# foobaz/pngloss

Measured on AMD Instinct MI355X. Metric: Mpixels/s (filter+quantise path), 4096x4096 RGBA8 s=19; bit-exact vs ref, higher is better.
Workload: dtype u8

## Files before the change

pngloss_amd/csrc/pl_seg_core.h:

```cpp
#ifndef PL_SEG_CORE_H
#define PL_SEG_CORE_H

#include <stdint.h>
#include <stddef.h>
#include <string.h>

#include "pl_result.h"

#if defined(__HIPCC__)
#define PLS_HD __host__ __device__ __forceinline__
#else
#define PLS_HD inline
#endif

#if defined(__HIP_DEVICE_COMPILE__)
#define PLS_THREADS(tid, nt) for (int tid = (int)threadIdx.x, pls_once_ = 1; pls_once_ && tid < (int)(nt); pls_once_ = 0)
#define PLS_SYNC() __syncthreads()
#define PLS_ATOMIC_ADD(p, v) atomicAdd((p), (v))
#define PLS_ATOMIC_MIN(p, v) atomicMin((p), (v))
#define PLS_ATOMIC_OR(p, v) atomicOr((p), (v))
#define PLS_ATOMIC_CAS(p, cmp, v) atomicCAS((p), (cmp), (v))
#define PLS_ATOMIC_ADD_RET(p, v) atomicAdd((p), (v))
#define PLS_ATOMIC_EXCH(p, v) atomicExch((p), (v))
#define PLS_ATOMIC_ADD64(p, v) atomicAdd((unsigned long long *)(p), (unsigned long long)(v))
// ... 92 lines not shown
#define SEG_UNC_SEEDS_OF(unit) ((unit) == 1 ? SEG_UNC_SEEDS1 : SEG_UNC_SEEDS)
#ifndef SEG_UNT
#define SEG_UNT 512
#endif
#define SEG_UPOOL SEG_UNT
#define SEG_GRP 16
#define SEG_VGRP 8
#define SEG_VGRP_UNITS 16
#ifndef SEG_TPARTS_BATCH
#define SEG_TPARTS_BATCH 1
#endif
#define SEG_VGRP_OF(tparts) ((tparts) == SEG_TPARTS_BATCH ? SEG_VGRP_UNITS : SEG_VGRP)
#define SEG_TPARTS 4
#define SEG_COMMIT_W 256
#define SEG_CTL_IMG_OF(P) (SEG_NFILT * (P).tparts)
#define SEG_PARTS 4
#define SEG_PL (SEG_L / SEG_PARTS)
#define SEG_NSP 256
#define SEG_NS_MAX 1024
#define SEG_TOFF 384
#define SEG_TN 768
#define SEG_TBL_WORDS (4 * SEG_TN + 128)
#define SEG_INVALID 0xFFFFu
#define SEG_NOFAIL 0xFFFFFFFFu
#define SEG_MAGIC 0x5E6C0DE1u
#define SEG_MAX_RESTARTS 12
#define SEG_NG_BURST 16
#define SEG_MAX_WIDTH (1u << 20)
#define SEG_THREADS 1024
#define SEG_CHAIN_THREADS 1024
#define SEG_CHAIN_THREADS_UNIT 256
#define SEG_REPLAY_THREADS (SEG_GRP * SEG_L)
// ... 600 lines not shown
    case 3: return seg_run_fast<3, TRX>(px, pstride, n, st, tw, cls, g, lut);
    case 4: return seg_run_fast<4, TRX>(px, pstride, n, st, tw, cls, g, lut);
    default: return seg_run_fast<0, TRX>(px, pstride, n, st, tw, cls, g, lut);
    }
}
PLS_HD int seg_run_fast_f(int f, bool trx, const SegPix *px, int pstride, int n, SegState &st, seg_lds_cu32 tw, seg_lds_cu8 cls, const SegGeo &g, seg_lds_cu32 lut)
{
    return trx ? seg_run_fast_t<true>(f, px, pstride, n, st, tw, cls, g, lut) : seg_run_fast_t<false>(f, px, pstride, n, st, tw, cls, g, lut);
}

#define SEG_K1 4
#ifndef SEG_K1_ONE_CHUNK
#define SEG_K1_ONE_CHUNK 4
#endif
PLS_HD int seg_k1(int ns) { return ns <= SEG_NSP ? SEG_K1_ONE_CHUNK : SEG_K1; }
#define SEG_HT 512
template <int NT>
PLS_HD void seg_enum_body(const SegJob &j, const SegParams &P, const SegCtlView &cv, int par, int f, int seg, int chalf, unsigned char *smem)
{
    if (cv.finished || cv.active != 1) return;
    const uint32_t W = j.W, bpp = j.bpp;
    constexpr int NCH = NT / SEG_NSP;
    const int c0 = chalf * NCH;
    if ((uint32_t)c0 >= bpp) return;
    const uint32_t x0 = (uint32_t)seg * SEG_L;
    if (x0 >= W) return;
    if (cv.start_x && x0 <= cv.start_x) return;
    uint32_t *tw = (uint32_t *)smem;
    SegPix *px = (SegPix *)(smem + SEG_TBL_WORDS * 4);
    uint32_t *lut = (uint32_t *)(px + (SEG_L + 1) * 4);
// ... 90 lines not shown
    PLS_THREADS(tid, NT) {
        uint32_t Dc[NCH];
        for (int k = 0; k < NCH; k++) Dc[k] = trflag[1 + k] < SEG_NSP ? trflag[1 + k] : SEG_NSP;
        int lc = 0, i = tid;
        uint32_t D = Dc[0];
        PLS_UNROLL
        for (int k = 0; k + 1 < NCH; k++) if (lc == k && (uint32_t)i >= Dc[k]) { i -= (int)Dc[k]; lc = k + 1; D = Dc[k + 1]; }
        const int c = c0 + lc;
        if (tid < NCH && (uint32_t)(c0 + tid) < bpp) j.dcnt[((size_t)f * j.nseg + seg) * 4 + c0 + tid] = trflag[1 + tid] < SEG_NSP ? trflag[1 + tid] : SEG_NSP;
        if ((uint32_t)c < bpp && (uint32_t)i < D) {
            const uint32_t key = uniq[lc * SEG_NSP + i];
            SegState st;
            st.left = (int)(key & 255u); st.cn = seg_sext8((int)(key >> 8)); st.th = seg_sext8((int)(key >> 16));
            uint32_t out = SEG_INVALID;
            const size_t slot = (((size_t)f * j.nseg + seg) * 4 + c) * SEG_NSP + i;
            int bad = seg_run_fast_f(f, trx, px + (1 + K1) * 4 + c, 4, SEG_PL - K1, st, SEG_LDS_CU32(tw), SEG_LDS_CU8(tw + 4 * SEG_TN), G, SEG_LDS_CU32(lut));
            for (int part = 1; part < SEG_PARTS; part++) {
                j.rck[slot * (SEG_PARTS - 1) + (part - 1)] = bad ? 0xFFFFFFFFu : seg_state_pack(st);
                bad |= seg_run_fast_f(f, trx, px + (1 + part * SEG_PL) * 4 + c, 4, SEG_PL, st, SEG_LDS_CU32(tw), SEG_LDS_CU8(tw + 4 * SEG_TN), G, SEG_LDS_CU32(lut));
            }
            if (!bad) out = seg_state_encode(P, px[SEG_L * 4 + c], st);
            j.rout[slot] = (uint16_t)out;
            j.rst[slot] = bad ? 0xFFFFFFFFu : seg_state_pack(st);
        }
        if (prof && tid == 0) {
            te[3] = PLS_CLOCK(); te[4] = te[3];
            for (int q = 0; q < PLR_SEG_ENUM_PHASES; q++) { PLS_ATOMIC_MAX(&j.result[PLR_SEG_ENUM_MAX + q], (int32_t)(te[q + 1] - te[q])); PLS_ATOMIC_ADD((uint32_t *)&j.result[PLR_SEG_ENUM_SUM + q], (uint32_t)(te[q + 1] - te[q])); }
            PLS_ATOMIC_ADD((uint32_t *)&j.result[PLR_SEG_ENUM_RUNS], 1u);
            PLS_ATOMIC_ADD((uint32_t *)&j.result[PLR_SEG_ENUM_STATES], trflag[1] + trflag[2] + trflag[3] + trflag[4]);
        }
    }
}

#define SEG_SM_ENUM_SEEDED(nt) (SEG_TBL_WORDS * 4 + (SEG_KIN + SEG_L + 1) * 4 * 8 + 2048 + 32 + 4 * SEG_EH_WORDS * 4 + 4 * SEG_EH_WORDS * 2 + 4 * SEG_NSP * 4 + (nt) * 4 + 128)
// ... 166 lines not shown
    }
    PLS_THREADS(tid, NT) {
        uint32_t Dc[NCH];
        for (int k = 0; k < NCH; k++) Dc[k] = trflag[1 + k] < SEG_NSP ? trflag[1 + k] : SEG_NSP;
        int lc = 0, i = tid;
        uint32_t D = Dc[0];
        PLS_UNROLL
        for (int k = 0; k + 1 < NCH; k++) if (lc == k && (uint32_t)i >= Dc[k]) { i -= (int)Dc[k]; lc = k + 1; D = Dc[k + 1]; }
        const int c = c0 + lc;
        if (tid < NCH && (uint32_t)(c0 + tid) < bpp) j.dcnt[((size_t)f * j.nseg + seg) * 4 + c0 + tid] = trflag[1 + tid] < SEG_NSP ? trflag[1 + tid] : SEG_NSP;
        if ((uint32_t)c < bpp && (uint32_t)i < D) {
            SegState st = seg_eh_state(uniq[lc * SEG_NSP + i]);
            const size_t slot = (((size_t)f * j.nseg + seg) * 4 + c) * SEG_NSP + i;
            const SegPix *ps = px + (nrun + 1) * 4 + c;
            int bad = 0;
            for (int part = 0; part < SEG_PARTS; part++) {
                if (part) j.rck[slot * (SEG_PARTS - 1) + (part - 1)] = bad ? 0xFFFFFFFFu : seg_state_pack(st);
                bad |= seg_run_fast_f(f, trx, ps + part * SEG_PL * 4, 4, SEG_PL, st, SEG_LDS_CU32(tw), SEG_LDS_CU8(tw + 4 * SEG_TN), G, SEG_LDS_CU32(lut));
            }
            j.rst[slot] = bad ? 0xFFFFFFFFu : seg_state_pack(st);
        }
        if (prof && tid == 0) {
            te[3] = PLS_CLOCK(); te[4] = te[3];
            for (int q = 0; q < PLR_SEG_ENUM_PHASES; q++) { PLS_ATOMIC_MAX(&j.result[PLR_SEG_ENUM_MAX + q], (int32_t)(te[q + 1] - te[q])); PLS_ATOMIC_ADD((uint32_t *)&j.result[PLR_SEG_ENUM_SUM + q], (uint32_t)(te[q + 1] - te[q])); }
            PLS_ATOMIC_ADD((uint32_t *)&j.result[PLR_SEG_ENUM_RUNS], 1u);
            PLS_ATOMIC_ADD((uint32_t *)&j.result[PLR_SEG_ENUM_STATES], two_stage ? 2u * (trflag[1] + trflag[2]) : trflag[1] + trflag[2] + trflag[3] + trflag[4]);
        }
    }
}

template <int NT>
PLS_HD void seg_enum_small_body(const SegJob &j, const SegParams &P, const SegCtlView &cv, int par, int f, int seg0, unsigned char *smem)
{
// ... 22 lines not shown
        for (int q = 0; q < NTW; q++) { const int i = tid + q * NT; if (i < SEG_TBL_WORDS) tw[i] = vt[q]; }
        if (tid < 512) lut[tid] = vl;
        if (tid < NSEGS * SEG_L) {
            seg_pix_split4(px + tid * 4, vp, bpp, (uint32_t)seg0 * SEG_L + (uint32_t)tid, W);
            if ((bpp & 1u) == 0u && (px[tid * 4 + (bpp - 1u)].w >> 24)) PLS_ATOMIC_OR(trflag, 1u);
        }
    }
    PLS_SYNC();
    const bool trx = *trflag != 0u;
    PLS_THREADS(tid, NT) {
        const int sl = tid / (4 * SEG_NSS), c = (tid / SEG_NSS) & 3, i = tid % SEG_NSS;
        const uint32_t seg = (uint32_t)seg0 + (uint32_t)sl, x0 = seg * SEG_L;
        if (seg < j.nseg && x0 < W && (x0 > cv.start_x || cv.start_x == 0) && (uint32_t)c < bpp && i < P.ns_small) {
            SegState st;
            uint32_t out = SEG_INVALID;
            const size_t slot = (((size_t)f * j.nseg + seg) * 4 + c) * SEG_NSP + i;
            if (seg_small_decode(P, i, st)) {
                int bad = 0;
                for (int part = 0; part < SEG_PARTS; part++) {
                    if (part) j.rck[slot * (SEG_PARTS - 1) + (part - 1)] = bad ? 0xFFFFFFFFu : seg_state_pack(st);
                    bad |= seg_run_fast_f(f, trx, px + (sl * SEG_L + part * SEG_PL) * 4 + c, 4, SEG_PL, st, SEG_LDS_CU32(tw), SEG_LDS_CU8(tw + 4 * SEG_TN), G, SEG_LDS_CU32(lut));
                }
                if (!bad) out = seg_small_encode(P, st);
            } else {
                for (int part = 1; part < SEG_PARTS; part++) j.rck[slot * (SEG_PARTS - 1) + (part - 1)] = 0xFFFFFFFFu;
            }
            j.maps[(((size_t)f * j.nseg + seg) * 4 + c) * (size_t)P.nsp + i] = (uint16_t)i;
            j.rout[(((size_t)f * j.nseg + seg) * 4 + c) * SEG_NSP + i] = (uint16_t)out;
            j.rst[(((size_t)f * j.nseg + seg) * 4 + c) * SEG_NSP + i] = out == SEG_INVALID ? 0xFFFFFFFFu : seg_state_pack(st);
            if (i == 0) j.dcnt[((size_t)f * j.nseg + seg) * 4 + c] = (uint32_t)P.ns_small;
        }
    }
}

#ifndef SEG_UNC_SMALL
#define SEG_UNC_SMALL (SEG_UNIT <= 3 ? 20 : (SEG_UNIT <= 4 ? 15 : (SEG_UNIT <= 6 ? 10 : 7)))
#endif
#define SEG_UNC_SMALL_OF(unit) ((unit) == SEG_UNIT ? SEG_UNC_SMALL : (SEG_UNC_SMALL < 20 ? SEG_UNC_SMALL : 20))
#define SEG_UNPX (SEG_UNC_SMALL * (SEG_UNIT * SEG_L + 1))
#define SEG_UN_K1MAX 4
// ... 9 lines not shown
        uint32_t m = bits[w];
        if (w == (a >> 5)) m &= 0xFFFFFFFFu << (a & 31u);
        if (w == ((b - 1u) >> 5) && (b & 31u)) m &= 0xFFFFFFFFu >> (32u - (b & 31u));
        n += (uint32_t)__builtin_popcount(m);
    }
    return n;
}
template <int LANES, int UNIT, int NC, bool SEEDS = false>
PLS_HD void seg_enum_unit_body(const SegJob &j, const SegParams &P, const SegCtlView &cv, int par, int f, int grp, unsigned char *smem)
{
    if (cv.finished || cv.active != 1) return;
    constexpr int NT = SEG_UNT, HT = 2 * LANES;
    constexpr int CPR = NT / LANES < NC ? NT / LANES : NC;
    constexpr int ROUNDS = (NC + CPR - 1) / CPR;
    constexpr uint32_t E = UNIT, UL = E * SEG_L, NPX = UL + 1;
    static_assert(CPR * HT <= 2 * SEG_UNT && CPR * LANES <= SEG_UNT && NC <= 24 && NC * (UNIT * SEG_L + 1) <= SEG_UNPX, "hash tables, per-turn lists, pixel records and the bookkeeping words are sized for this");
    const uint32_t W = j.W, bpp = j.bpp, nseg = j.nseg, nunit = (nseg + E - 1) / E, ncombo = nunit * bpp;
    const uint32_t q0 = (uint32_t)grp * NC;
    if (q0 >= ncombo) return;
    const uint32_t sx = cv.start_x;
    { const uint32_t ql = seg_umin(q0 + NC, ncombo) - 1u; if (sx && (ql / bpp) * UL <= sx) return; }
    constexpr uint32_t NP1 = SEEDS ? SEG_SEED_KMAX + 1 : SEG_UN_K1MAX + 1;
    uint32_t *tw = (uint32_t *)smem;
    uint32_t *lut = tw + SEG_TBL_WORDS;
    uint32_t *pool = lut + 512;
    SegPix *px1_std = (SegPix *)(pool + SEG_UPOOL);
    uint32_t *misc = (uint32_t *)(px1_std + SEG_UNC_SMALL * (SEG_UN_K1MAX + 1));
    uint32_t *ht = misc + 128;
    uint16_t *dense = (uint16_t *)(ht + 2 * SEG_UNT);
    uint32_t *uniqr = (uint32_t *)(dense + 2 * SEG_UNT);
// ... 207 lines not shown
                for (uint32_t sg = u * E; sg < seg_umin(u * E + E, nseg); sg++) j.dcnt[((size_t)f * nseg + sg) * 4 + c] = D;
            }
        }
        if ((uint32_t)tid < total) {
            int k = 0;
            PLS_UNROLL
            for (int q = 1; q < NC; q++) k += (uint32_t)tid >= misc[32 + q] ? 1 : 0;
            const uint32_t i = (uint32_t)tid - misc[32 + k], cq = q0 + (uint32_t)k, u = cq / bpp, c = cq % bpp;
            const uint32_t key = pool[tid];
            SegState st;
            st.left = (int)(key & 255u); st.cn = seg_sext8((int)(key >> 8)); st.th = seg_sext8((int)(key >> 16));
            const SegPix *pk = px + (size_t)k * NPX;
            const uint32_t sg0 = u * E, nsg = seg_umin(E, nseg - sg0);
            const size_t slot = (((size_t)f * nseg + sg0) * 4 + c) * SEG_NSP + i;
            int bad = 0;
            for (int part = 0; part < SEG_PARTS; part++) {
                if (part) j.rck[slot * (SEG_PARTS - 1) + (part - 1)] = bad ? 0xFFFFFFFFu : seg_state_pack(st);
                const int skip = part == 0 ? K1 : 0;
                bad |= seg_run_fast_f(f, trx, pk + 1 + part * SEG_PL + skip, 1, SEG_PL - skip, st, SEG_LDS_CU32(tw), SEG_LDS_CU8(tw + 4 * SEG_TN), G, SEG_LDS_CU32(lut));
            }
            const uint32_t ps0 = bad ? 0xFFFFFFFFu : seg_state_pack(st);
            j.rst[slot] = ps0;
            SEG_DEBUG_STATE(f, (long)cv.y * 100000 + (long)cq, 0, i, ps0);
            if (nsg == 1u) j.rout[slot] = (uint16_t)(bad ? (uint32_t)SEG_INVALID : seg_any_encode(P, f, pk[SEG_L], st));
            pool[tid] = nsg > 1u ? ps0 : 0xFFFFFFFFu;
        }
    }
    if (prof) { PLS_SYNC(); te[3] = PLS_CLOCK(); }
    if (E > 1u) {
        PLS_SYNC();
        PLS_THREADS(tid, NT) {
            const uint32_t total = misc[32 + NC];
            if ((uint32_t)tid < total) {
                const uint32_t ps = pool[tid];
// ... 36 lines not shown
        }
        PLS_SYNC();
        PLS_THREADS(tid, NT) {
            const uint32_t total2 = misc[64 + NC];
            if ((uint32_t)tid < total2) {
                int k = 0;
                PLS_UNROLL
                for (int q = 1; q < NC; q++) k += (uint32_t)tid >= misc[64 + q] ? 1 : 0;
                const uint32_t i = (uint32_t)tid - misc[64 + k], cq = q0 + (uint32_t)k, u = cq / bpp, c = cq % bpp;
                SegState st = seg_state_unpack(pool2[misc[32 + k] + i]);
                const SegPix *pk = px + (size_t)k * NPX;
                const uint32_t sg0 = u * E, nsg = seg_umin(E, nseg - sg0);
                int bad = 0;
                for (uint32_t sl = 1; sl < nsg; sl++) {
                    const size_t slot = (((size_t)f * nseg + sg0 + sl) * 4 + c) * SEG_NSP + i;
                    for (int part = 0; part < SEG_PARTS; part++) {
                        if (part) j.rck[slot * (SEG_PARTS - 1) + (part - 1)] = bad ? 0xFFFFFFFFu : seg_state_pack(st);
                        bad |= seg_run_fast_f(f, trx, pk + 1 + sl * SEG_L + part * SEG_PL, 1, SEG_PL, st, SEG_LDS_CU32(tw), SEG_LDS_CU8(tw + 4 * SEG_TN), G, SEG_LDS_CU32(lut));
                    }
                    j.rst[slot] = bad ? 0xFFFFFFFFu : seg_state_pack(st);
                    SEG_DEBUG_STATE(f, (long)cv.y * 100000 + (long)cq, sl, i, bad ? 0xFFFFFFFFu : seg_state_pack(st));
                    if (sl + 1 == nsg) j.rout[slot] = (uint16_t)(bad ? (uint32_t)SEG_INVALID : seg_any_encode(P, f, pk[(sl + 1) * SEG_L], st));
                }
            }
        }
    }
    if (prof) {
        PLS_SYNC();
        PLS_THREADS(tid, NT) {
            if (tid == 0) {
                te[4] = PLS_CLOCK();
                for (int q = 0; q < PLR_SEG_ENUM_PHASES; q++) { PLS_ATOMIC_MAX(&j.result[PLR_SEG_ENUM_MAX + q], (int32_t)(te[q + 1] - te[q])); PLS_ATOMIC_ADD((uint32_t *)&j.result[PLR_SEG_ENUM_SUM + q], (uint32_t)(te[q + 1] - te[q])); }
                PLS_ATOMIC_ADD((uint32_t *)&j.result[PLR_SEG_ENUM_RUNS], 1u);
// ... 7 lines not shown
{
    return seeds != 0 && P.seed_n > 0 && !seg_is_small(P, f) && cv.start_x == 0u && j.nbreak * 16u <= cv.y + 128u;
}

PLS_HD void seg_load_frozen(const SegJob &j, int par, int f, uint32_t *Hf, uint32_t *rank, int tid, int nt)
{
    for (int b = tid; b < 256; b += nt) {
        Hf[b] = j.H0[par * 256 + b] + j.base[((size_t)par * SEG_NFILT + f) * 256 + b];
        rank[b] = j.orig_rank[f * 256 + b];
    }
}

PLS_HD void seg_cnt_add(uint32_t *cnt, int bin, uint32_t v) { PLS_ATOMIC_ADD(&cnt[bin >> 2], v << (8 * (bin & 3))); }
PLS_HD uint32_t seg_cnt_get(const uint32_t *cnt, int bin) { return (cnt[bin >> 2] >> (8 * (bin & 3))) & 255u; }
static_assert(SEG_L * 4 <= 255, "a segment's bump count of a bin fits a byte");
PLS_HD void seg_walk(int f, const SegPix *px, int pstride, uint32_t xa, uint32_t xe, SegState &st, seg_lds_cu32 tw, seg_lds_cu32 lut, const uint32_t *Hf,
                     const uint32_t *rank, const SegGeo &G, const uint32_t *lut_g, int bleed, uint32_t *out, uint32_t *cnt)
{
    const SegState st0 = st;
    int bad = 0;
    const seg_lds_cu8 cls = SEG_LDS_CU8(tw + 4 * SEG_TN);
    for (uint32_t x = xa; x < xe; x++) {
        uint32_t w;
        const SegPix &p = px[(size_t)(x - xa) * pstride];
        switch (f) {
        case 1: w = seg_step_fast<1, true>(p, st, bad, tw, cls, G, lut); break;
        case 2: w = seg_step_fast<2, true>(p, st, bad, tw, cls, G, lut); break;
        case 3: w = seg_step_fast<3, true>(p, st, bad, tw, cls, G, lut); break;
        case 4: w = seg_step_fast<4, true>(p, st, bad, tw, cls, G, lut); break;
        default: w = seg_step_fast<0, true>(p, st, bad, tw, cls, G, lut); break;
        }
        if (out) out[(size_t)(x - xa) * 4] = w;
        if (cnt) seg_cnt_add(cnt, seg_cand_bin(w), 1u);
    }
    if (seg_bad(bad)) {
        if (cnt && out) for (uint32_t x = xa; x < xe; x++) seg_cnt_add(cnt, seg_cand_bin(out[(size_t)(x - xa) * 4]), 0u - 1u);
        st = st0;
        for (uint32_t x = xa; x < xe; x++) {
            const uint32_t w = seg_step_scan(f, px[(size_t)(x - xa) * pstride], st, Hf, nullptr, rank, G, lut_g, bleed);
            if (out) out[(size_t)(x - xa) * 4] = w;
            if (cnt) seg_cnt_add(cnt, seg_cand_bin(w), 1u);
        }
    }
}

template <int NT, bool UNITS>
PLS_HD void seg_first_body(const SegJob &j, const SegParams &P, const SegCtlView &cv, int par, int f, unsigned char *smem)
{
    const SegCtl &ctl = j.ctl[par];
    if (cv.finished || cv.active != 1) return;
    const uint32_t W = j.W, bpp = j.bpp, nseg = j.nseg;
    const uint32_t sx = cv.start_x;
    if (sx >= W || sx == 0) return;
    const uint32_t first = sx / SEG_L;
    if (first + 1 >= nseg) return;
    const uint32_t E = UNITS ? seg_unit_of(P, f) : 1u, ulast = seg_umin((first / E) * E + E - 1u, nseg - 1u);
// ... 513 lines not shown
template <int RNT>
PLS_HD void seg_replay_body(const SegJob &j, const SegParams &P, const SegCtlView &cv, int par, int f, int grp, unsigned char *smem)
{
    const SegCtl &ctl = j.ctl[par];
    if (cv.finished) return;
    const bool lazy = f == 0 && cv.active == 2;
    if (!lazy && cv.active != 1) return;
    const uint32_t W = j.W, bpp = j.bpp, nseg = j.nseg;
    const uint32_t sx = cv.start_x;
    const uint32_t first = sx / SEG_L;
    const uint32_t seg0 = (uint32_t)grp * SEG_GRP, x0g = seg0 * SEG_L;
    const bool walk = !lazy && sx < W && seg0 + SEG_GRP > first;
    uint32_t *Hf = (uint32_t *)smem, *rank = Hf + 256, *lut = Hf + 512, *tw = Hf + 1024;
    SegPix *px = (SegPix *)(tw + SEG_TBL_WORDS);
    uint32_t *cnt = (uint32_t *)(px + SEG_GRP * SEG_L * 4);
    uint32_t *lane = cnt + SEG_GRP * 64;
    uint32_t *cwl = lane + SEG_GRP * SEG_PARTS * 4 * 2;
    uint32_t *oaL = cwl + SEG_REPLAY_THREADS * 4;
    uint32_t *rm = tw;
    uint32_t *red = rm + 768;
    uint32_t *h0s = red + 16;
    const uint32_t y = cv.y;
    const uint32_t *row = seg_row_orig(j, y), *nab = y ? j.img + (size_t)(y - 1u) * W : nullptr, *e0g = seg_e0(j, y);
    const uint32_t *oab = y ? seg_row_orig(j, y - 1u) : nullptr;
    const SegGeo G = seg_geo((int)cv.s);
    const bool adaptive = !j.row_filters || y == 0;
    PLS_THREADS(tid, RNT) {
        const bool walker = walk && tid < SEG_GRP * SEG_PARTS * 4;
        const int sl = tid / (SEG_PARTS * 4), part = (tid >> 2) % SEG_PARTS, c = tid & 3;
        const uint32_t sg = seg0 + (uint32_t)sl;
        const bool live = walker && sg < nseg && sg >= first && (uint32_t)c < bpp;
        const size_t sc = ((size_t)f * nseg + (live ? sg : 0u)) * 4 + c;
        const uint32_t d = live ? (uint32_t)j.dnout[sc] : SEG_INVALID;
        constexpr int NTW = (SEG_TBL_WORDS + RNT - 1) / RNT;
        uint32_t vt[NTW], vl = 0, vh = 0, vb = 0, vr = 0;
        PLS_UNROLL
        for (int q = 0; q < NTW; q++) { const int i = tid + q * RNT; vt[q] = (walk && i < SEG_TBL_WORDS) ? j.tables[(size_t)f * SEG_TBL_WORDS + i] : 0u; }
        if (walk && tid < 512) vl = P.lut_a[tid];
        if (walk && tid < 256) { vh = j.H0[par * 256 + tid]; vb = j.base[((size_t)par * SEG_NFILT + f) * 256 + tid]; vr = j.orig_rank[f * 256 + tid]; }
        const bool pixlane = tid < SEG_REPLAY_THREADS;
        const uint32_t x = pixlane ? x0g + (uint32_t)tid : W;
        const SegPixRaw vp = seg_pix_fetch(row, nab, e0g, x, W);
        const uint32_t voa = (!lazy && oab && x < W) ? oab[x] : 0u;
        uint32_t voa0 = 0, vol0 = 0;
        SegVec16 vw, vw0; vw.a = vw.b = vw.c = vw.d = 0u; vw0 = vw;
        if (!lazy && tid == 0 && x0g) { voa0 = oab ? oab[x0g - 1] : 0u; vol0 = row[x0g - 1]; if (x0g <= sx) vw0 = *(const SEG_AS_GLB SegVec16 *)(j.cand + ((size_t)f * W + x0g - 1) * 4); }
        if (!lazy && x < W && (x < sx || !walk)) vw = *(const SEG_AS_GLB SegVec16 *)(j.cand + ((size_t)f * W + x) * 4);
        uint32_t ck[SEG_PARTS - 1], ent = 0;
        PLS_UNROLL
        for (int q = 0; q < SEG_PARTS - 1; q++) ck[q] = 0xFFFFFFFFu;
        if (live) {
            if (d != SEG_INVALID && d < SEG_NSP) {
                PLS_UNROLL
                for (int q = 0; q < SEG_PARTS - 1; q++) ck[q] = j.rck[(sc * SEG_NSP + d) * (SEG_PARTS - 1) + q];
            }
            if (part == 0) ent = sg == first ? ctl.state[f][c] : j.entry[sc];
        }
        uint32_t st0 = 0, range = 0xFFFFFFFFu;
        if (live) {
            const uint32_t x0 = sg * SEG_L, xend = (uint32_t)seg_min((int)(x0 + SEG_L), (int)W);
            bool mine = part == 0;
            uint32_t xa = sg == first ? sx : x0;
            if (part == 0) st0 = ent;
            else {
                uint32_t ckp = 0xFFFFFFFFu;
                PLS_UNROLL
                for (int q = 0; q < SEG_PARTS - 1; q++) if (q == part - 1) ckp = ck[q];
                if (ckp != 0xFFFFFFFFu && x0 + (uint32_t)part * SEG_PL < xend && x0 + (uint32_t)part * SEG_PL > xa) { mine = true; st0 = ckp; xa = x0 + (uint32_t)part * SEG_PL; }
            }
            if (mine) {
                uint32_t xe = xend;
                PLS_UNROLL
                for (int q = SEG_PARTS - 1; q >= 1; q--)
                    if (q > part && ck[q - 1] != 0xFFFFFFFFu && x0 + (uint32_t)q * SEG_PL < xend && x0 + (uint32_t)q * SEG_PL > xa) xe = x0 + (uint32_t)q * SEG_PL;
                range = (xa - x0g) | ((xe - x0g) << 16);
                SEG_DEBUG_COUNT(part ? 1 : 0, xe - xa);
            }
        }
        if (tid < SEG_GRP * SEG_PARTS * 4) { lane[2 * tid] = st0; lane[2 * tid + 1] = range; }
        if (walk) {
            PLS_UNROLL
            for (int q = 0; q < NTW; q++) { const int i = tid + q * RNT; if (i < SEG_TBL_WORDS) tw[i] = vt[q]; }
            if (tid < 512) lut[tid] = vl;
            if (tid < 256) { Hf[tid] = vh + vb; rank[tid] = vr; }
            for (int i = tid; i < SEG_GRP * 64; i += RNT) cnt[i] = 0u;
        }
        if (pixlane) {
            seg_pix_split4(px + tid * 4, vp, bpp, x, W);
            oaL[tid + 1] = voa;
            cwl[tid * 4 + 0] = vw.a; cwl[tid * 4 + 1] = vw.b; cwl[tid * 4 + 2] = vw.c; cwl[tid * 4 + 3] = vw.d;
        }
        if (tid == 0) {
            oaL[0] = voa0; oaL[SEG_REPLAY_THREADS + 1] = vol0;
            oaL[SEG_REPLAY_THREADS + 2] = (vw0.a & 255u) | ((vw0.b & 255u) << 8) | ((vw0.c & 255u) << 16) | ((vw0.d & 255u) << 24);
        }
    }
    PLS_SYNC();
    if (walk) {
        PLS_THREADS(tid, RNT) {
            if (tid < SEG_GRP * SEG_PARTS * 4 && lane[2 * tid + 1] != 0xFFFFFFFFu) {
                const int sl = tid / (SEG_PARTS * 4), c = tid & 3;
                SegState st = seg_state_unpack(lane[2 * tid]);
                const uint32_t ra = lane[2 * tid + 1] & 0xffffu, re = lane[2 * tid + 1] >> 16;
                seg_walk(f, px + ra * 4 + c, 4, x0g + ra, x0g + re, st, SEG_LDS_CU32(tw), SEG_LDS_CU32(lut), Hf, rank, G, lut, P.bleed, cwl + ra * 4 + c, cnt + sl * 64);
            }
        }
        PLS_SYNC();
    }
    SegAcc &A = j.acc[par];
    PLS_THREADS(tid, RNT) { if (tid < 16) red[tid] = tid == 14 ? (0x80000000u ^ (uint32_t)(-(1 << 30))) : (tid == 15 ? (0x80000000u ^ (uint32_t)(1 << 30)) : 0u); }
    PLS_SYNC();
    {
        PLS_THREADS(tid, RNT) {
            if (walk && tid >= RNT - SEG_REPLAY_THREADS && tid < RNT - SEG_REPLAY_THREADS + 256) {
                const int b = tid - (RNT - SEG_REPLAY_THREADS);
                uint32_t tot = 0, cvs[SEG_GRP];
                PLS_UNROLL
                for (int sl = 0; sl < SEG_GRP; sl++) cvs[sl] = seg_cnt_get(cnt + sl * 64, b);
                PLS_UNROLL
                for (int sl = 0; sl < SEG_GRP; sl++) {
                    const uint32_t sg = seg0 + (uint32_t)sl;
                    if (sg < nseg && sg >= first) { j.segcnt[((size_t)f * nseg + sg) * 256 + b] = (uint16_t)cvs[sl]; tot += cvs[sl]; }
                }
                j.grpcnt[((size_t)f * j.ngrp + grp) * 256 + b] = tot;
            }
            const uint32_t x = (!lazy && tid < SEG_REPLAY_THREADS) ? x0g + (uint32_t)tid : W;
            uint64_t derr = 0; uint32_t hs[SEG_NFILT] = { 0, 0, 0, 0, 0 };
            if (x < W) {
                SegVec16 w; w.a = cwl[tid * 4 + 0]; w.b = cwl[tid * 4 + 1]; w.c = cwl[tid * 4 + 2]; w.d = cwl[tid * 4 + 3];
                if (walk && x >= sx) *(SEG_AS_GLB SegVec16 *)(j.cand + ((size_t)f * W + x) * 4) = w;
                uint32_t lw[4];
                if (tid) { PLS_UNROLL for (int c = 0; c < 4; c++) lw[c] = cwl[(tid - 1) * 4 + c] & 255u; }
                else {
                    uint32_t l0 = 0;
                    if (x0g && x0g <= sx) l0 = oaL[SEG_REPLAY_THREADS + 2];
                    else if (x0g) {
                        for (uint32_t c = 0; c < bpp; c++) l0 |= (walk ? (lane[2 * c] & 255u) : 0u) << (8 * c);
                        j.grpleft[(size_t)f * j.ngrp + grp] = l0;
                    }
                    PLS_UNROLL for (int c = 0; c < 4; c++) lw[c] = (l0 >> (8 * c)) & 255u;
                }
                const uint32_t wv[4] = { w.a, w.b, w.c, w.d };
                const uint32_t oav4 = oaL[tid + 1], odv4 = oaL[tid];
                for (uint32_t c = 0; c < bpp; c++) {
                    const int sh = 8 * (int)c;
                    const SegPix pc = px[tid * 4 + c];
                    const int back = (int)(wv[c] & 255u), nl = x ? (int)lw[c] : 0;
                    const int ov = (int)(pc.w & 255u), nav = (int)((pc.w >> 8) & 255u), ndv = (int)((pc.w >> 16) & 255u);
                    const int olv = tid ? (int)(px[(tid - 1) * 4 + c].w & 255u) : (int)((oaL[SEG_REPLAY_THREADS + 1] >> sh) & 255u);
                    const int oav = (int)((oav4 >> sh) & 255u), odv = (int)((odv4 >> sh) & 255u);
                    const int da = (oav - ov) - (nav - back), dd = (odv - ov) - (ndv - back), dl = (olv - ov) - (nl - back);
                    const uint32_t wgt = (bpp <= 2 && c == 0) ? 3u : 1u;
                    derr += (uint64_t)(wgt * (uint32_t)(da * da + dd * dd + dl * dl));
                    if (adaptive) {
                        const int preds[SEG_NFILT] = { 0, nl, nav, (nav + nl) >> 1, seg_paeth(nav, ndv, nl) };
                        for (int g = 0; g < SEG_NFILT; g++) { const int bb = (back - preds[g]) & 255; hs[g] += (uint32_t)(bb < 128 ? bb : 256 - bb); }
                    }
                }
            }
            derr = (uint64_t)pls_wave_sum_u32((uint32_t)derr);
            if (adaptive) for (int g = 0; g < SEG_NFILT; g++) hs[g] = pls_wave_sum_u32(hs[g]);
            if (PLS_WAVE_LEADER(tid)) {
                PLS_ATOMIC_ADD64((uint64_t *)&red[0], derr);
                if (adaptive) for (int g = 0; g < SEG_NFILT; g++) PLS_ATOMIC_ADD(&red[2 + g], hs[g]);
            }
        }
    }
    int R = -1;
    if (f == 0 && j.rowmm) {
        const int32_t *rmm = seg_rowmm(j, y);
        PLS_THREADS(tid, RNT) {
// ... 30 lines not shown
                        if (pc.w >> 24) hmax = h0s[0];
                        else hmax = rm[seg_min(seg_max((int)(pc.w & 255u) + pc.e0, -256), 511) + 256];
                        const uint32_t fr = hmax + rowbumps;
                        lb += 33u + (uint32_t)__builtin_clz(fr ? fr : 1u);
                    }
                }
                lb = pls_wave_sum_u64(lb);
                if (PLS_WAVE_LEADER(tid) && lb) PLS_ATOMIC_ADD64((uint64_t *)&red[10], lb);
            }
        }
    }
    PLS_SYNC();
    PLS_THREADS(tid, RNT) {
        if (tid == 0) {
            if (!lazy) {
                PLS_ATOMIC_ADD64(&A.derr[f], *(uint64_t *)&red[0]);
                if (adaptive) for (int g = 0; g < SEG_NFILT; g++) PLS_ATOMIC_ADD(&A.hs[f][g], red[2 + g]);
            }
            if (f == 0 && R >= 0) { PLS_ATOMIC_ADD64(&A.none_lb, *(uint64_t *)&red[10]); PLS_ATOMIC_ADD(&A.lb_valid, 1u); }
        }
    }
}

struct SegVal {
    const uint32_t *cw, *ro, *na, *e0, *lut, *H0, *rank, *cum;
    uint32_t bpp, sx, xg0, W;
    int f, bleed;
    SegGeo G;
    uint32_t *wbits;
    const uint8_t *slot_of;
    const uint32_t *pcw;
    uint32_t pc_stride;
// ... 911 lines not shown
```

Baseline: 92.69.

## Split segment walks into more checkpointed parts and fuse error sums into walker

Raises the number of checkpoint parts per segment from four to eight for the single-unit and full replay paths, so more walker threads can resume mid-segment in parallel. The distortion and filter-heuristic sums are now accumulated inside the walk itself, and the later per-pixel pass only applies a correction at lane starts where the assumed left neighbour differs. This aims to cut serial walk length and the redundant second sweep. The cost is more checkpoint storage and writes in rck, extra per-step arithmetic and registers in the walker, and correction atomics that add complexity.

```diff
diff --git a/pngloss_amd/csrc/pl_seg_core.h b/pngloss_amd/csrc/pl_seg_core.h
--- a/pngloss_amd/csrc/pl_seg_core.h
+++ b/pngloss_amd/csrc/pl_seg_core.h
@@ -130,8 +130,10 @@
 #define SEG_TPARTS 4
 #define SEG_COMMIT_W 256
 #define SEG_CTL_IMG_OF(P) (SEG_NFILT * (P).tparts)
-#define SEG_PARTS 4
-#define SEG_PL (SEG_L / SEG_PARTS)
+#define SEG_PARTS 8
+#define SEG_PARTS_UNITS 4
+#define SEG_PARTS_OF_UNIT(unit) ((unit) == 1 ? SEG_PARTS : SEG_PARTS_UNITS)
+#define SEG_PARTS_OF_REPLAY(rnt) ((rnt) == SEG_REPLAY_NT ? SEG_PARTS : SEG_PARTS_UNITS)
 #define SEG_NSP 256
 #define SEG_NS_MAX 1024
 #define SEG_TOFF 384
@@ -762,6 +764,8 @@
 #define SEG_K1_ONE_CHUNK 4
 #endif
 PLS_HD int seg_k1(int ns) { return ns <= SEG_NSP ? SEG_K1_ONE_CHUNK : SEG_K1; }
+static_assert(SEG_L % SEG_PARTS == 0 && SEG_L % SEG_PARTS_UNITS == 0 && SEG_PARTS_UNITS <= SEG_PARTS, "parts of whole pixels; rck has room for the larger count");
+static_assert(SEG_K1 <= SEG_L / SEG_PARTS && SEG_K1_ONE_CHUNK <= SEG_L / SEG_PARTS, "the dedupe lies in part 0: the distinct states run SEG_L / parts - K1 >= 0 steps to the first checkpoint");
 #define SEG_HT 512
 template <int NT>
 PLS_HD void seg_enum_body(const SegJob &j, const SegParams &P, const SegCtlView &cv, int par, int f, int seg, int chalf, unsigned char *smem)
@@ -882,10 +886,11 @@
             st.left = (int)(key & 255u); st.cn = seg_sext8((int)(key >> 8)); st.th = seg_sext8((int)(key >> 16));
             uint32_t out = SEG_INVALID;
             const size_t slot = (((size_t)f * j.nseg + seg) * 4 + c) * SEG_NSP + i;
-            int bad = seg_run_fast_f(f, trx, px + (1 + K1) * 4 + c, 4, SEG_PL - K1, st, SEG_LDS_CU32(tw), SEG_LDS_CU8(tw + 4 * SEG_TN), G, SEG_LDS_CU32(lut));
-            for (int part = 1; part < SEG_PARTS; part++) {
-                j.rck[slot * (SEG_PARTS - 1) + (part - 1)] = bad ? 0xFFFFFFFFu : seg_state_pack(st);
-                bad |= seg_run_fast_f(f, trx, px + (1 + part * SEG_PL) * 4 + c, 4, SEG_PL, st, SEG_LDS_CU32(tw), SEG_LDS_CU8(tw + 4 * SEG_TN), G, SEG_LDS_CU32(lut));
+            constexpr int PARTS = SEG_PARTS, PL = SEG_L / PARTS;
+            int bad = seg_run_fast_f(f, trx, px + (1 + K1) * 4 + c, 4, PL - K1, st, SEG_LDS_CU32(tw), SEG_LDS_CU8(tw + 4 * SEG_TN), G, SEG_LDS_CU32(lut));
+            for (int part = 1; part < PARTS; part++) {
+                j.rck[slot * (PARTS - 1) + (part - 1)] = bad ? 0xFFFFFFFFu : seg_state_pack(st);
+                bad |= seg_run_fast_f(f, trx, px + (1 + part * PL) * 4 + c, 4, PL, st, SEG_LDS_CU32(tw), SEG_LDS_CU8(tw + 4 * SEG_TN), G, SEG_LDS_CU32(lut));
             }
             if (!bad) out = seg_state_encode(P, px[SEG_L * 4 + c], st);
             j.rout[slot] = (uint16_t)out;
@@ -1082,9 +1087,10 @@
             const size_t slot = (((size_t)f * j.nseg + seg) * 4 + c) * SEG_NSP + i;
             const SegPix *ps = px + (nrun + 1) * 4 + c;
             int bad = 0;
-            for (int part = 0; part < SEG_PARTS; part++) {
-                if (part) j.rck[slot * (SEG_PARTS - 1) + (part - 1)] = bad ? 0xFFFFFFFFu : seg_state_pack(st);
-                bad |= seg_run_fast_f(f, trx, ps + part * SEG_PL * 4, 4, SEG_PL, st, SEG_LDS_CU32(tw), SEG_LDS_CU8(tw + 4 * SEG_TN), G, SEG_LDS_CU32(lut));
+            constexpr int PARTS = SEG_PARTS, PL = SEG_L / PARTS;
+            for (int part = 0; part < PARTS; part++) {
+                if (part) j.rck[slot * (PARTS - 1) + (part - 1)] = bad ? 0xFFFFFFFFu : seg_state_pack(st);
+                bad |= seg_run_fast_f(f, trx, ps + part * PL * 4, 4, PL, st, SEG_LDS_CU32(tw), SEG_LDS_CU8(tw + 4 * SEG_TN), G, SEG_LDS_CU32(lut));
             }
             j.rst[slot] = bad ? 0xFFFFFFFFu : seg_state_pack(st);
         }
@@ -1137,16 +1143,17 @@
         if (seg < j.nseg && x0 < W && (x0 > cv.start_x || cv.start_x == 0) && (uint32_t)c < bpp && i < P.ns_small) {
             SegState st;
             uint32_t out = SEG_INVALID;
+            constexpr int PARTS = SEG_PARTS, PL = SEG_L / PARTS;
             const size_t slot = (((size_t)f * j.nseg + seg) * 4 + c) * SEG_NSP + i;
             if (seg_small_decode(P, i, st)) {
                 int bad = 0;
-                for (int part = 0; part < SEG_PARTS; part++) {
-                    if (part) j.rck[slot * (SEG_PARTS - 1) + (part - 1)] = bad ? 0xFFFFFFFFu : seg_state_pack(st);
-                    bad |= seg_run_fast_f(f, trx, px + (sl * SEG_L + part * SEG_PL) * 4 + c, 4, SEG_PL, st, SEG_LDS_CU32(tw), SEG_LDS_CU8(tw + 4 * SEG_TN), G, SEG_LDS_CU32(lut));
+                for (int part = 0; part < PARTS; part++) {
+                    if (part) j.rck[slot * (PARTS - 1) + (part - 1)] = bad ? 0xFFFFFFFFu : seg_state_pack(st);
+                    bad |= seg_run_fast_f(f, trx, px + (sl * SEG_L + part * PL) * 4 + c, 4, PL, st, SEG_LDS_CU32(tw), SEG_LDS_CU8(tw + 4 * SEG_TN), G, SEG_LDS_CU32(lut));
                 }
                 if (!bad) out = seg_small_encode(P, st);
             } else {
-                for (int part = 1; part < SEG_PARTS; part++) j.rck[slot * (SEG_PARTS - 1) + (part - 1)] = 0xFFFFFFFFu;
+                for (int part = 1; part < PARTS; part++) j.rck[slot * (PARTS - 1) + (part - 1)] = 0xFFFFFFFFu;
             }
             j.maps[(((size_t)f * j.nseg + seg) * 4 + c) * (size_t)P.nsp + i] = (uint16_t)i;
             j.rout[(((size_t)f * j.nseg + seg) * 4 + c) * SEG_NSP + i] = (uint16_t)out;
@@ -1186,6 +1193,7 @@
     constexpr int CPR = NT / LANES < NC ? NT / LANES : NC;
     constexpr int ROUNDS = (NC + CPR - 1) / CPR;
     constexpr uint32_t E = UNIT, UL = E * SEG_L, NPX = UL + 1;
+    constexpr int PARTS = SEG_PARTS_OF_UNIT(UNIT), PL = SEG_L / PARTS;
     static_assert(CPR * HT <= 2 * SEG_UNT && CPR * LANES <= SEG_UNT && NC <= 24 && NC * (UNIT * SEG_L + 1) <= SEG_UNPX, "hash tables, per-turn lists, pixel records and the bookkeeping words are sized for this");
     const uint32_t W = j.W, bpp = j.bpp, nseg = j.nseg, nunit = (nseg + E - 1) / E, ncombo = nunit * bpp;
     const uint32_t q0 = (uint32_t)grp * NC;
@@ -1423,10 +1431,10 @@
             const uint32_t sg0 = u * E, nsg = seg_umin(E, nseg - sg0);
             const size_t slot = (((size_t)f * nseg + sg0) * 4 + c) * SEG_NSP + i;
             int bad = 0;
-            for (int part = 0; part < SEG_PARTS; part++) {
-                if (part) j.rck[slot * (SEG_PARTS - 1) + (part - 1)] = bad ? 0xFFFFFFFFu : seg_state_pack(st);
+            for (int part = 0; part < PARTS; part++) {
+                if (part) j.rck[slot * (PARTS - 1) + (part - 1)] = bad ? 0xFFFFFFFFu : seg_state_pack(st);
                 const int skip = part == 0 ? K1 : 0;
-                bad |= seg_run_fast_f(f, trx, pk + 1 + part * SEG_PL + skip, 1, SEG_PL - skip, st, SEG_LDS_CU32(tw), SEG_LDS_CU8(tw + 4 * SEG_TN), G, SEG_LDS_CU32(lut));
+                bad |= seg_run_fast_f(f, trx, pk + 1 + part * PL + skip, 1, PL - skip, st, SEG_LDS_CU32(tw), SEG_LDS_CU8(tw + 4 * SEG_TN), G, SEG_LDS_CU32(lut));
             }
             const uint32_t ps0 = bad ? 0xFFFFFFFFu : seg_state_pack(st);
             j.rst[slot] = ps0;
@@ -1493,9 +1501,9 @@
                 int bad = 0;
                 for (uint32_t sl = 1; sl < nsg; sl++) {
                     const size_t slot = (((size_t)f * nseg + sg0 + sl) * 4 + c) * SEG_NSP + i;
-                    for (int part = 0; part < SEG_PARTS; part++) {
-                        if (part) j.rck[slot * (SEG_PARTS - 1) + (part - 1)] = bad ? 0xFFFFFFFFu : seg_state_pack(st);
-                        bad |= seg_run_fast_f(f, trx, pk + 1 + sl * SEG_L + part * SEG_PL, 1, SEG_PL, st, SEG_LDS_CU32(tw), SEG_LDS_CU8(tw + 4 * SEG_TN), G, SEG_LDS_CU32(lut));
+                    for (int part = 0; part < PARTS; part++) {
+                        if (part) j.rck[slot * (PARTS - 1) + (part - 1)] = bad ? 0xFFFFFFFFu : seg_state_pack(st);
+                        bad |= seg_run_fast_f(f, trx, pk + 1 + sl * SEG_L + part * PL, 1, PL, st, SEG_LDS_CU32(tw), SEG_LDS_CU8(tw + 4 * SEG_TN), G, SEG_LDS_CU32(lut));
                     }
                     j.rst[slot] = bad ? 0xFFFFFFFFu : seg_state_pack(st);
                     SEG_DEBUG_STATE(f, (long)cv.y * 100000 + (long)cq, sl, i, bad ? 0xFFFFFFFFu : seg_state_pack(st));
@@ -1533,15 +1541,30 @@
 PLS_HD void seg_cnt_add(uint32_t *cnt, int bin, uint32_t v) { PLS_ATOMIC_ADD(&cnt[bin >> 2], v << (8 * (bin & 3))); }
 PLS_HD uint32_t seg_cnt_get(const uint32_t *cnt, int bin) { return (cnt[bin >> 2] >> (8 * (bin & 3))) & 255u; }
 static_assert(SEG_L * 4 <= 255, "a segment's bump count of a bin fits a byte");
+PLS_HD void seg_sum_add(uint32_t &derr, uint32_t *hs, bool adaptive, uint32_t wgt, int back, int nl, int nav, int ndv, int ov, int olv, int oav, int odv)
+{
+    const int da = (oav - ov) - (nav - back), dd = (odv - ov) - (ndv - back), dl = (olv - ov) - (nl - back);
+    derr += wgt * (uint32_t)(da * da + dd * dd + dl * dl);
+    if (adaptive) {
+        const int preds[SEG_NFILT] = { 0, nl, nav, (nav + nl) >> 1, seg_paeth(nav, ndv, nl) };
+        for (int g = 0; g < SEG_NFILT; g++) { const int bb = (back - preds[g]) & 255; hs[g] += (uint32_t)(bb < 128 ? bb : 256 - bb); }
+    }
+}
+struct SegWalkSums { const uint32_t *oa; int sh, olv; uint32_t wgt; bool adaptive; uint32_t derr, hs[SEG_NFILT]; };
+#define SEG_FLAG_WRONG_LEFT 8
 PLS_HD void seg_walk(int f, const SegPix *px, int pstride, uint32_t xa, uint32_t xe, SegState &st, seg_lds_cu32 tw, seg_lds_cu32 lut, const uint32_t *Hf,
-                     const uint32_t *rank, const SegGeo &G, const uint32_t *lut_g, int bleed, uint32_t *out, uint32_t *cnt)
+                     const uint32_t *rank, const SegGeo &G, const uint32_t *lut_g, int bleed, uint32_t *out, uint32_t *cnt, SegWalkSums *S = nullptr)
 {
     const SegState st0 = st;
     int bad = 0;
     const seg_lds_cu8 cls = SEG_LDS_CU8(tw + 4 * SEG_TN);
+    uint32_t oaw = S ? S->oa[0] : 0u;
+    int olv = S ? S->olv : 0;
     for (uint32_t x = xa; x < xe; x++) {
         uint32_t w;
         const SegPix &p = px[(size_t)(x - xa) * pstride];
+        const int nl = x ? st.left : 0;
+        const uint32_t oan = S ? S->oa[x - xa + 1] : 0u;
         switch (f) {
         case 1: w = seg_step_fast<1, true>(p, st, bad, tw, cls, G, lut); break;
         case 2: w = seg_step_fast<2, true>(p, st, bad, tw, cls, G, lut); break;
@@ -1551,14 +1574,29 @@
         }
         if (out) out[(size_t)(x - xa) * 4] = w;
         if (cnt) seg_cnt_add(cnt, seg_cand_bin(w), 1u);
+        if (S) {
+            const int ov = (int)(p.w & 255u);
+            seg_sum_add(S->derr, S->hs, S->adaptive, S->wgt, seg_cand_byte(w), nl, (int)((p.w >> 8) & 255u), (int)((p.w >> 16) & 255u), ov, olv,
+                        (int)((oan >> S->sh) & 255u), (int)((oaw >> S->sh) & 255u));
+            olv = ov; oaw = oan;
+        }
     }
     if (seg_bad(bad)) {
         if (cnt && out) for (uint32_t x = xa; x < xe; x++) seg_cnt_add(cnt, seg_cand_bin(out[(size_t)(x - xa) * 4]), 0u - 1u);
         st = st0;
+        if (S) { S->derr = 0u; for (int g = 0; g < SEG_NFILT; g++) S->hs[g] = 0u; olv = S->olv; }
         for (uint32_t x = xa; x < xe; x++) {
-            const uint32_t w = seg_step_scan(f, px[(size_t)(x - xa) * pstride], st, Hf, nullptr, rank, G, lut_g, bleed);
+            const SegPix &p = px[(size_t)(x - xa) * pstride];
+            const int nl = x ? st.left : 0;
+            const uint32_t w = seg_step_scan(f, p, st, Hf, nullptr, rank, G, lut_g, bleed);
             if (out) out[(size_t)(x - xa) * 4] = w;
             if (cnt) seg_cnt_add(cnt, seg_cand_bin(w), 1u);
+            if (S) {
+                const int ov = (int)(p.w & 255u);
+                seg_sum_add(S->derr, S->hs, S->adaptive, S->wgt, seg_cand_byte(w), nl, (int)((p.w >> 8) & 255u), (int)((p.w >> 16) & 255u), ov, olv,
+                            (int)((S->oa[x - xa + 1] >> S->sh) & 255u), (int)((S->oa[x - xa] >> S->sh) & 255u));
+                olv = ov;
+            }
         }
     }
 }
@@ -2102,9 +2140,15 @@
     uint32_t *Hf = (uint32_t *)smem, *rank = Hf + 256, *lut = Hf + 512, *tw = Hf + 1024;
     SegPix *px = (SegPix *)(tw + SEG_TBL_WORDS);
     uint32_t *cnt = (uint32_t *)(px + SEG_GRP * SEG_L * 4);
+    constexpr int PARTS = SEG_PARTS_OF_REPLAY(RNT), PL = SEG_L / PARTS, NWALK = SEG_GRP * PARTS * 4;
+    static_assert(NWALK <= RNT && NWALK <= SEG_GRP * SEG_PARTS * 4, "a thread per walker; `lane` is carved for SEG_PARTS parts");
+    constexpr bool WSUMS = RNT == SEG_REPLAY_NT;
     uint32_t *lane = cnt + SEG_GRP * 64;
     uint32_t *cwl = lane + SEG_GRP * SEG_PARTS * 4 * 2;
     uint32_t *oaL = cwl + SEG_REPLAY_THREADS * 4;
+    uint32_t *wsum = oaL + SEG_REPLAY_THREADS + 4;
+    static_assert((1024 + SEG_TBL_WORDS + SEG_GRP * SEG_L * 4 * 2 + SEG_GRP * 64 + SEG_GRP * SEG_PARTS * 4 * 2 + SEG_REPLAY_THREADS * 4 + SEG_REPLAY_THREADS + 4 + 8) * 4 <= SEG_SM_REPLAY
+                  && (1024 + SEG_TBL_WORDS + SEG_GRP * SEG_L * 4 * 2 + SEG_GRP * 64 + SEG_GRP * SEG_PARTS * 4 * 2 + SEG_REPLAY_THREADS * 4 + SEG_REPLAY_THREADS + 4) % 2 == 0, "the carve ends within the kernel's LDS request");
     uint32_t *rm = tw;
     uint32_t *red = rm + 768;
     uint32_t *h0s = red + 16;
@@ -2114,8 +2158,8 @@
     const SegGeo G = seg_geo((int)cv.s);
     const bool adaptive = !j.row_filters || y == 0;
     PLS_THREADS(tid, RNT) {
-        const bool walker = walk && tid < SEG_GRP * SEG_PARTS * 4;
-        const int sl = tid / (SEG_PARTS * 4), part = (tid >> 2) % SEG_PARTS, c = tid & 3;
+        const bool walker = walk && tid < NWALK;
+        const int sl = tid / (PARTS * 4), part = (tid >> 2) % PARTS, c = tid & 3;
         const uint32_t sg = seg0 + (uint32_t)sl;
         const bool live = walker && sg < nseg && sg >= first && (uint32_t)c < bpp;
         const size_t sc = ((size_t)f * nseg + (live ? sg : 0u)) * 4 + c;
@@ -2134,13 +2178,13 @@
         SegVec16 vw, vw0; vw.a = vw.b = vw.c = vw.d = 0u; vw0 = vw;
         if (!lazy && tid == 0 && x0g) { voa0 = oab ? oab[x0g - 1] : 0u; vol0 = row[x0g - 1]; if (x0g <= sx) vw0 = *(const SEG_AS_GLB SegVec16 *)(j.cand + ((size_t)f * W + x0g - 1) * 4); }
         if (!lazy && x < W && (x < sx || !walk)) vw = *(const SEG_AS_GLB SegVec16 *)(j.cand + ((size_t)f * W + x) * 4);
-        uint32_t ck[SEG_PARTS - 1], ent = 0;
+        uint32_t ck[PARTS - 1], ent = 0;
         PLS_UNROLL
-        for (int q = 0; q < SEG_PARTS - 1; q++) ck[q] = 0xFFFFFFFFu;
+        for (int q = 0; q < PARTS - 1; q++) ck[q] = 0xFFFFFFFFu;
         if (live) {
             if (d != SEG_INVALID && d < SEG_NSP) {
                 PLS_UNROLL
-                for (int q = 0; q < SEG_PARTS - 1; q++) ck[q] = j.rck[(sc * SEG_NSP + d) * (SEG_PARTS - 1) + q];
+                for (int q = 0; q < PARTS - 1; q++) ck[q] = j.rck[(sc * SEG_NSP + d) * (PARTS - 1) + q];
             }
             if (part == 0) ent = sg == first ? ctl.state[f][c] : j.entry[sc];
         }
@@ -2153,19 +2197,19 @@
             else {
                 uint32_t ckp = 0xFFFFFFFFu;
                 PLS_UNROLL
-                for (int q = 0; q < SEG_PARTS - 1; q++) if (q == part - 1) ckp = ck[q];
-                if (ckp != 0xFFFFFFFFu && x0 + (uint32_t)part * SEG_PL < xend && x0 + (uint32_t)part * SEG_PL > xa) { mine = true; st0 = ckp; xa = x0 + (uint32_t)part * SEG_PL; }
+                for (int q = 0; q < PARTS - 1; q++) if (q == part - 1) ckp = ck[q];
+                if (ckp != 0xFFFFFFFFu && x0 + (uint32_t)part * PL < xend && x0 + (uint32_t)part * PL > xa) { mine = true; st0 = ckp; xa = x0 + (uint32_t)part * PL; }
             }
             if (mine) {
                 uint32_t xe = xend;
                 PLS_UNROLL
-                for (int q = SEG_PARTS - 1; q >= 1; q--)
-                    if (q > part && ck[q - 1] != 0xFFFFFFFFu && x0 + (uint32_t)q * SEG_PL < xend && x0 + (uint32_t)q * SEG_PL > xa) xe = x0 + (uint32_t)q * SEG_PL;
+                for (int q = PARTS - 1; q >= 1; q--)
+                    if (q > part && ck[q - 1] != 0xFFFFFFFFu && x0 + (uint32_t)q * PL < xend && x0 + (uint32_t)q * PL > xa) xe = x0 + (uint32_t)q * PL;
                 range = (xa - x0g) | ((xe - x0g) << 16);
                 SEG_DEBUG_COUNT(part ? 1 : 0, xe - xa);
             }
         }
-        if (tid < SEG_GRP * SEG_PARTS * 4) { lane[2 * tid] = st0; lane[2 * tid + 1] = range; }
+        if (tid < NWALK) { lane[2 * tid] = st0; lane[2 * tid + 1] = range; }
         if (walk) {
             PLS_UNROLL
             for (int q = 0; q < NTW; q++) { const int i = tid + q * RNT; if (i < SEG_TBL_WORDS) tw[i] = vt[q]; }
@@ -2178,6 +2222,7 @@
             oaL[tid + 1] = voa;
             cwl[tid * 4 + 0] = vw.a; cwl[tid * 4 + 1] = vw.b; cwl[tid * 4 + 2] = vw.c; cwl[tid * 4 + 3] = vw.d;
         }
+        if (tid < 8) wsum[tid] = 0u;
         if (tid == 0) {
             oaL[0] = voa0; oaL[SEG_REPLAY_THREADS + 1] = vol0;
             oaL[SEG_REPLAY_THREADS + 2] = (vw0.a & 255u) | ((vw0.b & 255u) << 8) | ((vw0.c & 255u) << 16) | ((vw0.d & 255u) << 24);
@@ -2186,11 +2231,38 @@
     PLS_SYNC();
     if (walk) {
         PLS_THREADS(tid, RNT) {
-            if (tid < SEG_GRP * SEG_PARTS * 4 && lane[2 * tid + 1] != 0xFFFFFFFFu) {
-                const int sl = tid / (SEG_PARTS * 4), c = tid & 3;
-                SegState st = seg_state_unpack(lane[2 * tid]);
-                const uint32_t ra = lane[2 * tid + 1] & 0xffffu, re = lane[2 * tid + 1] >> 16;
-                seg_walk(f, px + ra * 4 + c, 4, x0g + ra, x0g + re, st, SEG_LDS_CU32(tw), SEG_LDS_CU32(lut), Hf, rank, G, lut, P.bleed, cwl + ra * 4 + c, cnt + sl * 64);
+            if (tid < NWALK) {
+                SegWalkSums S;
+                S.derr = 0u;
+                for (int g = 0; g < SEG_NFILT; g++) S.hs[g] = 0u;
+                if (lane[2 * tid + 1] != 0xFFFFFFFFu) {
+                    const int sl = tid / (PARTS * 4), c = tid & 3;
+                    SegState st = seg_state_unpack(lane[2 * tid]);
+                    const uint32_t ra = lane[2 * tid + 1] & 0xffffu, re = lane[2 * tid + 1] >> 16;
+                    S.oa = oaL + ra; S.sh = 8 * c; S.wgt = (bpp <= 2 && c == 0) ? 3u : 1u; S.adaptive = adaptive;
+                    S.olv = (int)((ra ? px[(ra - 1) * 4 + c].w : (oaL[SEG_REPLAY_THREADS + 1] >> S.sh)) & 255u);
+#if !defined(__HIP_DEVICE_COMPILE__)
+                    const int nl0 = st.left;
+#endif
+                    seg_walk(f, px + ra * 4 + c, 4, x0g + ra, x0g + re, st, SEG_LDS_CU32(tw), SEG_LDS_CU32(lut), Hf, rank, G, lut, P.bleed, cwl + ra * 4 + c, cnt + sl * 64, WSUMS ? &S : nullptr);
+#if !defined(__HIP_DEVICE_COMPILE__)
+                    if (WSUMS && (P.engine_flags & SEG_FLAG_WRONG_LEFT) && x0g + ra && (ra || x0g <= sx)) {
+                        const SegPix pc = px[ra * 4 + c];
+                        uint32_t dr = 0, dw = 0, hr[SEG_NFILT] = { 0, 0, 0, 0, 0 }, hw[SEG_NFILT] = { 0, 0, 0, 0, 0 };
+                        for (int wrong = 0; wrong < 2; wrong++)
+                            seg_sum_add(wrong ? dw : dr, wrong ? hw : hr, adaptive, S.wgt, seg_cand_byte(cwl[ra * 4 + c]), nl0 ^ (wrong ? 255 : 0), (int)((pc.w >> 8) & 255u), (int)((pc.w >> 16) & 255u), (int)(pc.w & 255u), S.olv,
+                                        (int)((oaL[ra + 1] >> S.sh) & 255u), (int)((oaL[ra] >> S.sh) & 255u));
+                        S.derr += dw - dr;
+                        for (int g = 0; g < SEG_NFILT; g++) S.hs[g] += hw[g] - hr[g];
+                    }
+#endif
+                }
+                if (WSUMS) S.derr = pls_wave_sum_u32(S.derr);
+                if (WSUMS && adaptive) for (int g = 0; g < SEG_NFILT; g++) S.hs[g] = pls_wave_sum_u32(S.hs[g]);
+                if (WSUMS && PLS_WAVE_LEADER(tid)) {
+                    PLS_ATOMIC_ADD64((uint64_t *)&wsum[0], (uint64_t)S.derr);
+                    if (adaptive) for (int g = 0; g < SEG_NFILT; g++) PLS_ATOMIC_ADD(&wsum[2 + g], S.hs[g]);
+                }
             }
         }
         PLS_SYNC();
@@ -2216,6 +2288,7 @@
             uint64_t derr = 0; uint32_t hs[SEG_NFILT] = { 0, 0, 0, 0, 0 };
             if (x < W) {
                 SegVec16 w; w.a = cwl[tid * 4 + 0]; w.b = cwl[tid * 4 + 1]; w.c = cwl[tid * 4 + 2]; w.d = cwl[tid * 4 + 3];
+                const bool walked = WSUMS && walk && x >= sx;
                 if (walk && x >= sx) *(SEG_AS_GLB SegVec16 *)(j.cand + ((size_t)f * W + x) * 4) = w;
                 uint32_t lw[4];
                 if (tid) { PLS_UNROLL for (int c = 0; c < 4; c++) lw[c] = cwl[(tid - 1) * 4 + c] & 255u; }
@@ -2230,19 +2303,34 @@
                 }
                 const uint32_t wv[4] = { w.a, w.b, w.c, w.d };
                 const uint32_t oav4 = oaL[tid + 1], odv4 = oaL[tid];
+                const int kseg = tid / SEG_L, kin = tid % SEG_L;
+                const bool at_sx = x == sx;
+                const bool lane_start = walked && x && (at_sx || kin % PL == 0) && (tid || x0g <= sx);
+                const int l4 = (kseg * PARTS + (at_sx ? 0 : kin / PL)) * 4;
                 for (uint32_t c = 0; c < bpp; c++) {
                     const int sh = 8 * (int)c;
+                    int nl = x ? (int)lw[c] : 0, nlw = nl;
+                    if (walked) {
+                        if (!lane_start || lane[2 * (l4 + (int)c) + 1] == 0xFFFFFFFFu || (lane[2 * (l4 + (int)c) + 1] & 0xffffu) != (uint32_t)tid) continue;
+                        nlw = (int)(lane[2 * (l4 + (int)c)] & 255u);
+#if !defined(__HIP_DEVICE_COMPILE__)
+                        if (P.engine_flags & SEG_FLAG_WRONG_LEFT) nlw ^= 255;
+#endif
+                        if (nlw == nl) continue;
+                    }
                     const SegPix pc = px[tid * 4 + c];
-                    const int back = (int)(wv[c] & 255u), nl = x ? (int)lw[c] : 0;
+                    const int back = (int)(wv[c] & 255u);
                     const int ov = (int)(pc.w & 255u), nav = (int)((pc.w >> 8) & 255u), ndv = (int)((pc.w >> 16) & 255u);
                     const int olv = tid ? (int)(px[(tid - 1) * 4 + c].w & 255u) : (int)((oaL[SEG_REPLAY_THREADS + 1] >> sh) & 255u);
                     const int oav = (int)((oav4 >> sh) & 255u), odv = (int)((odv4 >> sh) & 255u);
-                    const int da = (oav - ov) - (nav - back), dd = (odv - ov) - (ndv - back), dl = (olv - ov) - (nl - back);
                     const uint32_t wgt = (bpp <= 2 && c == 0) ? 3u : 1u;
-                    derr += (uint64_t)(wgt * (uint32_t)(da * da + dd * dd + dl * dl));
-                    if (adaptive) {
-                        const int preds[SEG_NFILT] = { 0, nl, nav, (nav + nl) >> 1, seg_paeth(nav, ndv, nl) };
-                        for (int g = 0; g < SEG_NFILT; g++) { const int bb = (back - preds[g]) & 255; hs[g] += (uint32_t)(bb < 128 ? bb : 256 - bb); }
+                    if (!walked) { uint32_t d32 = 0; seg_sum_add(d32, hs, adaptive, wgt, back, nl, nav, ndv, ov, olv, oav, odv); derr += (uint64_t)d32; }
+                    else {
+                        uint32_t dr = 0, dw = 0, hr[SEG_NFILT] = { 0, 0, 0, 0, 0 }, hw[SEG_NFILT] = { 0, 0, 0, 0, 0 };
+                        seg_sum_add(dr, hr, adaptive, wgt, back, nl, nav, ndv, ov, olv, oav, odv);
+                        seg_sum_add(dw, hw, adaptive, wgt, back, nlw, nav, ndv, ov, olv, oav, odv);
+                        PLS_ATOMIC_ADD64((uint64_t *)&wsum[0], (uint64_t)dr - (uint64_t)dw);
+                        if (adaptive) for (int g = 0; g < SEG_NFILT; g++) PLS_ATOMIC_ADD(&wsum[2 + g], hr[g] - hw[g]);
                     }
                 }
             }
@@ -2303,8 +2391,8 @@
     PLS_THREADS(tid, RNT) {
         if (tid == 0) {
             if (!lazy) {
-                PLS_ATOMIC_ADD64(&A.derr[f], *(uint64_t *)&red[0]);
-                if (adaptive) for (int g = 0; g < SEG_NFILT; g++) PLS_ATOMIC_ADD(&A.hs[f][g], red[2 + g]);
+                PLS_ATOMIC_ADD64(&A.derr[f], *(uint64_t *)&red[0] + *(uint64_t *)&wsum[0]);
+                if (adaptive) for (int g = 0; g < SEG_NFILT; g++) PLS_ATOMIC_ADD(&A.hs[f][g], red[2 + g] + wsum[2 + g]);
             }
             if (f == 0 && R >= 0) { PLS_ATOMIC_ADD64(&A.none_lb, *(uint64_t *)&red[10]); PLS_ATOMIC_ADD(&A.lb_valid, 1u); }
         }
```

After: 90.30. 2.6% lower.
